# callmeray/PointMVSNet

Measured on AMD Instinct MI355X. Metric: depth-maps/sec (DTU 640x512, 3 src views, 2 flow iters), higher is better.
Workload: dtype f32

## Files before the change

### pointmvsnet_amd/csrc/conv2d_wide.hip

```cpp
#include <stdlib.h>

#include "pf_common.h"
#include "pf_bn_resolve.h"

namespace {

typedef float f32x16 __attribute__((ext_vector_type(16)));
typedef float f32x4 __attribute__((ext_vector_type(4)));
typedef float f32x2 __attribute__((ext_vector_type(2)));

struct WideGeom {
  int Hi, Wi, Ho, Wo, tiles_w, tiles_h, sps;
  int cl_out;
  int sets, spset, x_mode;
  int64_t w_stride;
};

__device__ __forceinline__ int wide_set(const WideGeom& g, int n) { return (g.sets > 1 && n >= g.spset) ? 1 : 0; }
__device__ __forceinline__ int wide_input_sample(const WideGeom& g, int n, int set) {
  const int i = n - set * g.spset;
  return g.x_mode == 0 ? n : (g.x_mode == 1 ? i : i * g.sets + set);
}

template <int KS, int STRIDE, int CIN, int COUT>
struct WideCfg {
  static constexpr int NWN = COUT / 32;
  static constexpr int NWM = 4 / NWN;
  static constexpr int TH = 2 * NWM, TW = 16;
  static constexpr int PAD = KS / 2;
  static constexpr int PH = (TH - 1) * STRIDE + KS, PW = (TW - 1) * STRIDE + KS;
  static constexpr int NPIX = PH * PW;
  static constexpr int RS = CIN + 4;
  static constexpr int PATCH = NPIX * RS;
  static constexpr int KC = CIN / 8;
  static constexpr size_t LDS = sizeof(float) * (size_t)(PATCH + 2 * CIN) + sizeof(double) * 4 * 32 * 2;
  static_assert(COUT == 32 || COUT == 64, "C_out is 32 or 64");
  static_assert(CIN % 8 == 0 && PATCH % 4 == 0, "16-byte pieces");
  static_assert(PATCH * sizeof(float) >= 4096, "pf_bn_resolve's scratch lives in the (still empty) patch");
  static_assert(LDS <= 80 * 1024, "two blocks per CU");
};

template <int CIN, int NPIX, int PW, int RS>
struct PatchStager {
  static constexpr int ITEMS = NPIX * ((CIN + 3) / 4);
  static constexpr int NIT = (ITEMS + 255) / 256;
  static constexpr int PH = NPIX / PW;
  static_assert(CIN % 4 == 0 || CIN < 4, "a padded quad: one quad only");
  static_assert(PH < 256 && PW < 256, "patch coordinates are packed in bytes");
  float rx[NIT][4];
  int goff[NIT];
  int meta[NIT];
  unsigned okmask;
  bool interior;

  __device__ __forceinline__ void init(int plane_i, int Wi) {
    const int tid = threadIdx.x;
#pragma unroll
    for (int r = 0; r < NIT; ++r) {
      const int it = tid + 256 * r;
      const int itc = it < ITEMS ? it : ITEMS - 1;
      const int q = itc / NPIX, p = itc - q * NPIX;
      const int pr = p / PW, pc = p - pr * PW;
      goff[r] = 4 * q * plane_i + pr * Wi + pc;
      meta[r] = pr | (pc << 8) | (q << 16);
    }
  }

  __device__ __forceinline__ void load(const float* __restrict__ xb, int plane_i, int ih0, int iw0, int Hi, int Wi) {
    interior = ih0 >= 0 && iw0 >= 0 && ih0 + PH <= Hi && iw0 + PW <= Wi;
    const int origin = ih0 * Wi + iw0;
    if (interior) {
      okmask = ~0u;
#pragma unroll
      for (int r = 0; r < NIT; ++r) {
        const float* src = xb + (goff[r] + origin);
#pragma unroll
        for (int j = 0; j < 4; ++j) rx[r][j] = (CIN % 4 == 0 || j < CIN) ? src[j * plane_i] : 0.0f;
      }
      return;
    }
    okmask = 0;
#pragma unroll
    for (int r = 0; r < NIT; ++r) {
      const int pr = meta[r] & 255, pc = (meta[r] >> 8) & 255, q = meta[r] >> 16;
      const int ih = ih0 + pr, iw = iw0 + pc;
      const bool ok = ih >= 0 && ih < Hi && iw >= 0 && iw < Wi;
      okmask |= (ok ? 1u : 0u) << r;
      const float* src = xb + (ok ? goff[r] + origin : 4 * q * plane_i);
#pragma unroll
      for (int j = 0; j < 4; ++j) rx[r][j] = (CIN % 4 == 0 || j < CIN) ? src[j * plane_i] : 0.0f;
    }
  }

  template <bool AFF>
  __device__ __forceinline__ void commit(float* patch, const float* aff) const {
    const int tid = threadIdx.x;
#pragma unroll
    for (int r = 0; r < NIT; ++r) {
      const int it = tid + 256 * r;
      const int pr = meta[r] & 255, pc = (meta[r] >> 8) & 255, q = meta[r] >> 16;
      f32x4 v = {rx[r][0], rx[r][1], rx[r][2], rx[r][3]};
      if (AFF) {
        const f32x4 a = *reinterpret_cast<const f32x4*>(aff + 4 * q);
        const f32x4 b = *reinterpret_cast<const f32x4*>(aff + CIN + 4 * q);
#pragma unroll
        for (int j = 0; j < 4; ++j) v[j] = fmaxf(fmaf(v[j], a[j], b[j]), 0.0f);
      }
      if (!interior && !((okmask >> r) & 1u)) v = (f32x4){0.0f, 0.0f, 0.0f, 0.0f};
      if (256 * (r + 1) <= ITEMS || it < ITEMS) *reinterpret_cast<f32x4*>(patch + (pr * PW + pc) * RS + 4 * q) = v;
    }
  }
};

template <int CIN, int AFFINE>
__device__ __forceinline__ void wide_affine_prologue(float* aff, const float* __restrict__ in_scale,
                                                     const float* __restrict__ in_shift, int stat,
                                                     const pf_bn_job& in_bn, double* scratch) {
  static_assert(CIN % 4 == 0 || AFFINE == 0, "a padded channel quad takes no affine");
  const int tid = threadIdx.x;
  if (AFFINE == 1) {
    const float* sc = in_scale + (int64_t)stat * CIN;
    const float* sh = in_shift + (int64_t)stat * CIN;
    if (tid < CIN) aff[tid] = sc[tid];
    else if (tid < 2 * CIN) aff[tid] = sh[tid - CIN];
    __syncthreads();
  }
  if (AFFINE == 2) pf_bn_resolve<256>(in_bn, stat, aff, aff + CIN, scratch);
}

template <int CIN, int NPIX, int PW, int RS, int AFFINE>
__device__ __forceinline__ void wide_stage_patch(const float* __restrict__ xb, int plane_i, int ih0, int iw0, int Hi,
                                                 int Wi, float* patch, float* aff, const float* __restrict__ in_scale,
                                                 const float* __restrict__ in_shift, int stat, const pf_bn_job& in_bn,
                                                 double* scratch) {
  PatchStager<CIN, NPIX, PW, RS> st;
  st.init(plane_i, Wi);
  st.load(xb, plane_i, ih0, iw0, Hi, Wi);
  wide_affine_prologue<CIN, AFFINE>(aff, in_scale, in_shift, stat, in_bn, scratch);
  st.template commit<(AFFINE != 0)>(patch, aff);
}

template <class C, int COUT>
__device__ __forceinline__ void wide_epilogue(const f32x16& acc, float* __restrict__ y, const WideGeom& g,
                                              double* __restrict__ partials, double* red, int n, int bx, int oh0,
                                              int ow0, int wm, int wn, int wave, int m, int h, int tid, bool cl_out) {
  const int co = wn * 32 + m;
  float* yb = y + ((int64_t)n * COUT + co) * ((int64_t)g.Ho * g.Wo);
  const bool vec_ok = (g.Wo & 3) == 0;
  float s = 0.0f, q = 0.0f;
  if (cl_out) {
    float* ycl = y + (int64_t)n * g.Ho * g.Wo * COUT + co;
#pragma unroll
    for (int rq = 0; rq < 4; ++rq) {
      const int oh = oh0 + 2 * wm + (rq >> 1);
      const int ow = ow0 + (rq & 1) * 8 + 4 * h;
      if (oh < g.Ho) {
#pragma unroll
        for (int e = 0; e < 4; ++e) {
          if (ow + e < g.Wo) {
            ycl[((int64_t)oh * g.Wo + ow + e) * COUT] = acc[4 * rq + e];
            s += acc[4 * rq + e];
            q += acc[4 * rq + e] * acc[4 * rq + e];
          }
        }
      }
    }
  } else
#pragma unroll
  for (int rq = 0; rq < 4; ++rq) {
    const int oh = oh0 + 2 * wm + (rq >> 1);
    const int ow = ow0 + (rq & 1) * 8 + 4 * h;
    if (oh < g.Ho) {
      float* dst = yb + (int64_t)oh * g.Wo + ow;
      if (vec_ok && ow + 3 < g.Wo) {
        *reinterpret_cast<float4*>(dst) = make_float4(acc[4 * rq], acc[4 * rq + 1], acc[4 * rq + 2], acc[4 * rq + 3]);
#pragma unroll
        for (int e = 0; e < 4; ++e) {
          s += acc[4 * rq + e];
          q += acc[4 * rq + e] * acc[4 * rq + e];
        }
      } else {
#pragma unroll
        for (int e = 0; e < 4; ++e) {
          if (ow + e < g.Wo) {
            dst[e] = acc[4 * rq + e];
            s += acc[4 * rq + e];
            q += acc[4 * rq + e] * acc[4 * rq + e];
          }
        }
      }
    }
  }
  if (partials != nullptr) {
    s += __shfl_xor(s, 32);
    q += __shfl_xor(q, 32);
    if (h == 0) {
      red[(wave * 32 + m) * 2 + 0] = (double)s;
      red[(wave * 32 + m) * 2 + 1] = (double)q;
    }
    __syncthreads();
    if (tid < COUT) {
      const int cn = tid >> 5, cm = tid & 31;
      double ds = 0.0, dq = 0.0;
#pragma unroll
      for (int w = 0; w < C::NWM; ++w) {
        ds += red[((w * C::NWN + cn) * 32 + cm) * 2 + 0];
        dq += red[((w * C::NWN + cn) * 32 + cm) * 2 + 1];
      }
      double* o = partials + (((int64_t)n * gridDim.x + bx) * COUT + tid) * 2;
      o[0] = ds;
      o[1] = dq;
    }
  }
}


template <int KS, int STRIDE, int CIN, int COUT, int AFFINE>
__global__ __launch_bounds__(256) void conv2d_wide_kernel(const float* __restrict__ x, const float* __restrict__ wp,
                                                            float* __restrict__ y, WideGeom g,
                                                            const float* __restrict__ in_scale,
                                                            const float* __restrict__ in_shift,
                                                            double* __restrict__ partials, pf_bn_job in_bn,
                                                            pf_bn_job in_bn1) {
  using C = WideCfg<KS, STRIDE, CIN, COUT>;
  constexpr int PW = C::PW, RS = C::RS, NPIX = C::NPIX;
  extern __shared__ __attribute__((aligned(16))) float lds[];
  float* patch = lds;
  float* aff = lds + C::PATCH;
  double* red = reinterpret_cast<double*>(aff + 2 * CIN);

  const int tid = threadIdx.x;
  const int wave = __builtin_amdgcn_readfirstlane(tid >> 6), lane = tid & 63;
  const int m = lane & 31, h = lane >> 5;
  const int wm = wave / C::NWN, wn = wave % C::NWN;
  unsigned xb_, xn_;
  pf_xcd_xy(xb_, xn_);
  const int n = (int)xn_, bx = (int)xb_;
  const int tw = bx % g.tiles_w, th = bx / g.tiles_w;
  const int oh0 = th * C::TH, ow0 = tw * C::TW;
  const int ih0 = oh0 * STRIDE - C::PAD, iw0 = ow0 * STRIDE - C::PAD;
  const int plane_i = g.Hi * g.Wi;
  const int set = wide_set(g, n);
  const float* xb = x + (int64_t)wide_input_sample(g, n, set) * CIN * plane_i;

  constexpr int NP = KS * KS * C::KC;
  constexpr int D = 6;
  const f32x4* bg = reinterpret_cast<const f32x4*>(wp + set * g.w_stride) + (h * COUT + wn * 32 + m);
  f32x4 bq[D];
#pragma unroll
  for (int d = 0; d < D; ++d) bq[d] = bg[(d < NP ? d : 0) * 2 * COUT];

  wide_stage_patch<CIN, NPIX, PW, RS, AFFINE>(xb, plane_i, ih0, iw0, g.Hi, g.Wi, patch, aff, in_scale, in_shift,
                                              AFFINE == 2 ? (n - set * g.spset) / g.sps : n / g.sps,
                                              set ? in_bn1 : in_bn, reinterpret_cast<double*>(patch));
  __syncthreads();

  f32x16 acc;
#pragma unroll
  for (int i = 0; i < 16; ++i) acc[i] = 0.0f;
  const float* abase = patch + ((2 * wm + (m >> 4)) * STRIDE * PW + (m & 15) * STRIDE) * RS + 4 * h;
  f32x4 a = *reinterpret_cast<const f32x4*>(abase);
#pragma unroll
  for (int t = 0; t < NP; ++t) {
    f32x4 an = a;
    if (t + 1 < NP) {
      const int tap = (t + 1) / C::KC, kc = (t + 1) % C::KC;
      const int kh = tap / KS, kw = tap % KS;
      an = *reinterpret_cast<const f32x4*>(abase + (kh * PW + kw) * RS + 8 * kc);
    }
    const f32x4 b = bq[t % D];
    __builtin_amdgcn_sched_barrier(0);
    acc = __builtin_amdgcn_mfma_f32_32x32x2f32(a.x, b.x, acc, 0, 0, 0);
    acc = __builtin_amdgcn_mfma_f32_32x32x2f32(a.y, b.y, acc, 0, 0, 0);
    acc = __builtin_amdgcn_mfma_f32_32x32x2f32(a.z, b.z, acc, 0, 0, 0);
    acc = __builtin_amdgcn_mfma_f32_32x32x2f32(a.w, b.w, acc, 0, 0, 0);
    __builtin_amdgcn_sched_barrier(0);
    if (t + D < NP) bq[t % D] = bg[(t + D) * 2 * COUT];
    a = an;
  }
  wide_epilogue<C, COUT>(acc, y, g, partials, red, n, bx, oh0, ow0, wm, wn, wave, m, h, tid, (g.cl_out >> set) & 1);
}

template <int KS, int STRIDE, int CIN, int COUT, int AFFINE>
int launch_wide_mode(const float* x, const float* wp, float* y, WideGeom g, int64_t N, const float* in_scale,
                     const float* in_shift, double* partials, const pf_bn_job& in_bn, const pf_bn_job& in_bn1,
                     hipStream_t s) {
  using C = WideCfg<KS, STRIDE, CIN, COUT>;
  if (C::LDS > 64 * 1024) {
    static std::atomic<unsigned long long> done{0};
    const int rc = pf_allow_big_lds(reinterpret_cast<const void*>(&conv2d_wide_kernel<KS, STRIDE, CIN, COUT, AFFINE>),
                                    (int)C::LDS, done);
    if (rc != PF_OK) return rc;
  }
  g.tiles_w = (g.Wo + C::TW - 1) / C::TW;
  const int tiles_h = (g.Ho + C::TH - 1) / C::TH;
  dim3 grid((unsigned)(tiles_h * g.tiles_w), (unsigned)N);
  hipLaunchKernelGGL((conv2d_wide_kernel<KS, STRIDE, CIN, COUT, AFFINE>), grid, dim3(256), C::LDS, s, x, wp, y, g,
                     in_scale, in_shift, partials, in_bn, in_bn1);
  return pf_launch_status();
}

template <int KS, int STRIDE, int CIN, int COUT>
int launch_wide(const float* x, const float* wp, float* y, WideGeom g, int64_t N, const float* in_scale,
                const float* in_shift, double* partials, const pf_bn_job* in_bn, hipStream_t s) {
  if (in_bn != nullptr) {
    for (int k = 0; k < g.sets; ++k) {
      const int rc = pf_bn_in_check(in_bn + k, CIN, g.spset / g.sps);
      if (rc != PF_OK) return rc;
    }
    return launch_wide_mode<KS, STRIDE, CIN, COUT, 2>(x, wp, y, g, N, nullptr, nullptr, partials, in_bn[0],
                                                      in_bn[g.sets - 1], s);
  }
  pf_bn_job none = {};
  if (in_scale != nullptr)
    return launch_wide_mode<KS, STRIDE, CIN, COUT, 1>(x, wp, y, g, N, in_scale, in_shift, partials, none, none, s);
  return launch_wide_mode<KS, STRIDE, CIN, COUT, 0>(x, wp, y, g, N, nullptr, nullptr, partials, none, none, s);
}

template <int KS, int STRIDE, int CIN, int COUT>
struct Wide16Cfg {
  static constexpr int TH = 16, TW = 16, NCOL = 16;
  static constexpr int PAD = KS / 2;
  static constexpr int PH = (TH - 1) * STRIDE + KS, PW = (TW - 1) * STRIDE + KS;
  static constexpr int NPIX = PH * PW;
  static constexpr int CINP = (CIN + 3) / 4 * 4;
  static constexpr int RS = CINP + 4;
  static constexpr int PATCH = NPIX * RS;
  static constexpr int CPL = CINP / 4;
  static constexpr bool PAIR = COUT == 8 && CIN >= 8;
  static constexpr int KH = PAIR ? KS + 1 : KS;
  static constexpr int WALL = KH * KS * CINP * NCOL;
  static constexpr int WSPACE = WALL > 1024 ? WALL : 1024;
  static constexpr size_t LDS = sizeof(float) * (size_t)(PATCH + WSPACE + 2 * CINP) + sizeof(double) * 4 * 16 * 2;
  static_assert(CIN == 3 || CIN == 8 || CIN == 16, "C_in is 3, 8 or 16");
  static_assert(COUT == 8 || COUT == 16, "C_out is 8 or 16");
  static_assert(!PAIR || STRIDE == 1, "paired rows: stride 1");
  static_assert(PATCH % 4 == 0 && WALL % 4 == 0, "16-byte pieces");
  static_assert(LDS <= 80 * 1024, "two blocks per CU");
};

template <int KS, int STRIDE, int CIN, int COUT, int AFFINE>
__global__ __launch_bounds__(256) void conv2d_wide16_kernel(const float* __restrict__ x, const float* __restrict__ wp,
                                                            float* __restrict__ y, WideGeom g,
                                                            const float* __restrict__ in_scale,
                                                            const float* __restrict__ in_shift,
                                                            double* __restrict__ partials, pf_bn_job in_bn,
                                                            pf_bn_job in_bn1) {
  using C = Wide16Cfg<KS, STRIDE, CIN, COUT>;
  constexpr int PW = C::PW, RS = C::RS, NPIX = C::NPIX, CPL = C::CPL, NCOL = 16;
  extern __shared__ __attribute__((aligned(16))) float lds[];
  float* patch = lds;
  float* wl = lds + C::PATCH;
  float* aff = wl + C::WSPACE;
  double* red = reinterpret_cast<double*>(aff + 2 * C::CINP);

  const int tid = threadIdx.x;
  const int wave = __builtin_amdgcn_readfirstlane(tid >> 6), lane = tid & 63;
  const int li = lane & 15, kq = lane >> 4;
  unsigned xb_, xn_;
  pf_xcd_xy(xb_, xn_);
  const int n = (int)xn_, bx = (int)xb_;
  const int plane_i = g.Hi * g.Wi;
  const int set = wide_set(g, n);
  const float* xb = x + (int64_t)wide_input_sample(g, n, set) * CIN * plane_i;
  wp += set * g.w_stride;
  const int tiles = g.tiles_h * g.tiles_w;
  const int nb = gridDim.x;

  constexpr int W4 = C::WALL / 4, NWR = (W4 + 255) / 256;
  f32x4 rw[NWR];
#pragma unroll
  for (int r = 0; r < NWR; ++r) {
    const int e = tid + 256 * r;
    rw[r] = reinterpret_cast<const f32x4*>(wp)[e < W4 ? e : W4 - 1];
  }
  PatchStager<CIN, NPIX, PW, RS> st;
  st.init(plane_i, g.Wi);
  int tile = bx;
  auto tile_origin = [&](int t, int& oh0, int& ow0) {
    const int th = t / g.tiles_w;
    oh0 = th * C::TH;
    ow0 = (t - th * g.tiles_w) * C::TW;
  };
  {
    int oh0, ow0;
    tile_origin(tile, oh0, ow0);
    st.load(xb, plane_i, oh0 * STRIDE - C::PAD, ow0 * STRIDE - C::PAD, g.Hi, g.Wi);
  }
  wide_affine_prologue<CIN, AFFINE>(aff, in_scale, in_shift, AFFINE == 2 ? (n - set * g.spset) / g.sps : n / g.sps,
                                    set ? in_bn1 : in_bn, reinterpret_cast<double*>(wl));
#pragma unroll
  for (int r = 0; r < NWR; ++r) {
    const int e = tid + 256 * r;
    if (256 * (r + 1) <= W4 || e < W4) reinterpret_cast<f32x4*>(wl)[e] = rw[r];
  }

  constexpr bool PAIR = C::PAIR;
  constexpr int NR = PAIR ? 2 : 4;
  const float* abase = patch + ((4 * wave) * STRIDE * PW + li * STRIDE) * RS + CPL * kq;
  const float* bbase = wl + (kq * NCOL + li) * CPL;
  constexpr int TAPS = C::KH * KS;
  struct Op {
    float v[CPL];
  };
  auto read_op = [&](const float* p) {
    Op o;
    if (CPL == 4) {
      const f32x4 t = *reinterpret_cast<const f32x4*>(p);
      o.v[0] = t[0];
      o.v[1 % CPL] = t[1];
      o.v[2 % CPL] = t[2];
      o.v[3 % CPL] = t[3];
    } else if (CPL == 2) {
      const f32x2 t = *reinterpret_cast<const f32x2*>(p);
      o.v[0] = t[0];
      o.v[1 % CPL] = t[1];
    } else {
      o.v[0] = p[0];
    }
    return o;
  };
  auto read_a = [&](int t, Op* a) {
    const int kh = t / KS, kw = t - kh * KS;
#pragma unroll
    for (int r = 0; r < NR; ++r) a[r] = read_op(abase + (((PAIR ? 2 * r : r) * STRIDE + kh) * PW + kw) * RS);
  };
  const bool vec_ok = (g.Wo & 3) == 0;
  const int my_co = PAIR ? (li & 7) : li;
  const int my_row = PAIR ? (li >> 3) : 0;
  const bool col_ok = my_co < COUT;
  const int plane_o = g.Ho * g.Wo;
  float* const yn = y + (int64_t)n * COUT * plane_o;
  double ds = 0.0, dq = 0.0;
#pragma unroll 1
  for (; tile < tiles; tile += nb) {
    int oh0, ow0;
    tile_origin(tile, oh0, ow0);
    st.template commit<(AFFINE != 0)>(patch, aff);
    __syncthreads();
    if (tile + nb < tiles) {
      int noh0, now0;
      tile_origin(tile + nb, noh0, now0);
      st.load(xb, plane_i, noh0 * STRIDE - C::PAD, now0 * STRIDE - C::PAD, g.Hi, g.Wi);
    }
    f32x4 acc[NR];
#pragma unroll
    for (int r = 0; r < NR; ++r) acc[r] = (f32x4){0.0f, 0.0f, 0.0f, 0.0f};
    Op a[NR], b;
    read_a(0, a);
    b = read_op(bbase);
#pragma unroll
    for (int t = 0; t < TAPS; ++t) {
      Op an[NR], bn = b;
#pragma unroll
      for (int r = 0; r < NR; ++r) an[r] = a[r];
      if (t + 1 < TAPS) {
        read_a(t + 1, an);
        bn = read_op(bbase + (t + 1) * 4 * NCOL * CPL);
      }
      __builtin_amdgcn_sched_barrier(0);
#pragma unroll
      for (int j = 0; j < CPL; ++j)
#pragma unroll
        for (int r = 0; r < NR; ++r) acc[r] = __builtin_amdgcn_mfma_f32_16x16x4f32(a[r].v[j], b.v[j], acc[r], 0, 0, 0);
      __builtin_amdgcn_sched_barrier(0);
#pragma unroll
      for (int r = 0; r < NR; ++r) a[r] = an[r];
      b = bn;
    }
    float s = 0.0f, q = 0.0f;
    const int ow = ow0 + 4 * kq;
    if (vec_ok && oh0 + C::TH <= g.Ho && ow0 + C::TW <= g.Wo) {
      float* dst = yn + (my_co * plane_o + (oh0 + 4 * wave + my_row) * g.Wo + ow);
      if (col_ok) {
#pragma unroll
        for (int r = 0; r < NR; ++r) {
          *reinterpret_cast<f32x4*>(dst + (PAIR ? 2 * r : r) * g.Wo) = acc[r];
#pragma unroll
          for (int e = 0; e < 4; ++e) {
            s += acc[r][e];
            q += acc[r][e] * acc[r][e];
          }
        }
      }
    } else {
      float* yb = yn + (int64_t)my_co * plane_o;
#pragma unroll
      for (int r = 0; r < NR; ++r) {
        const int oh = oh0 + 4 * wave + (PAIR ? 2 * r : r) + my_row;
        if (oh < g.Ho && col_ok) {
          float* dst = yb + (int64_t)oh * g.Wo + ow;
#pragma unroll
          for (int e = 0; e < 4; ++e) {
            if (ow + e < g.Wo) {
              dst[e] = acc[r][e];
              s += acc[r][e];
              q += acc[r][e] * acc[r][e];
            }
          }
        }
      }
    }
    ds += (double)s;
    dq += (double)q;
    __syncthreads();
  }
  if (PAIR && partials != nullptr) {
    ds += __shfl_xor(ds, 8);
    dq += __shfl_xor(dq, 8);
  }
  if (partials != nullptr) {
    ds += __shfl_xor(ds, 16);
    dq += __shfl_xor(dq, 16);
    ds += __shfl_xor(ds, 32);
    dq += __shfl_xor(dq, 32);
    if (lane < 16) {
      red[(wave * 16 + lane) * 2 + 0] = ds;
      red[(wave * 16 + lane) * 2 + 1] = dq;
    }
    __syncthreads();
    if (tid < COUT) {
      double ts = 0.0, tq = 0.0;
#pragma unroll
      for (int w = 0; w < 4; ++w) {
        ts += red[(w * 16 + tid) * 2 + 0];
        tq += red[(w * 16 + tid) * 2 + 1];
      }
      double* o = partials + (((int64_t)n * gridDim.x + bx) * COUT + tid) * 2;
      o[0] = ts;
      o[1] = tq;
    }
  }
}

#ifndef PF_W16_TPB
#define PF_W16_TPB 4
#endif
int wide16_blocks(int tiles) { return (tiles + PF_W16_TPB - 1) / PF_W16_TPB; }

template <int KS, int STRIDE, int CIN, int COUT, int AFFINE>
int launch_wide16_mode(const float* x, const float* wp, float* y, WideGeom g, int64_t N, const float* in_scale,
                       const float* in_shift, double* partials, const pf_bn_job& in_bn, const pf_bn_job& in_bn1,
                       hipStream_t s) {
  using C = Wide16Cfg<KS, STRIDE, CIN, COUT>;
  if (C::LDS > 64 * 1024) {
    static std::atomic<unsigned long long> done{0};
    const int rc = pf_allow_big_lds(
        reinterpret_cast<const void*>(&conv2d_wide16_kernel<KS, STRIDE, CIN, COUT, AFFINE>), (int)C::LDS, done);
    if (rc != PF_OK) return rc;
  }
  g.tiles_w = (g.Wo + C::TW - 1) / C::TW;
  g.tiles_h = (g.Ho + C::TH - 1) / C::TH;
  dim3 grid((unsigned)wide16_blocks(g.tiles_h * g.tiles_w), (unsigned)N);
  hipLaunchKernelGGL((conv2d_wide16_kernel<KS, STRIDE, CIN, COUT, AFFINE>), grid, dim3(256), C::LDS, s, x, wp, y, g,
                     in_scale, in_shift, partials, in_bn, in_bn1);
  return pf_launch_status();
}

template <int KS, int STRIDE, int CIN, int COUT>
int launch_wide16(const float* x, const float* wp, float* y, WideGeom g, int64_t N, const float* in_scale,
                  const float* in_shift, double* partials, const pf_bn_job* in_bn, hipStream_t s) {
  pf_bn_job none = {};
  if constexpr (CIN % 4 == 0) {
    if (in_bn != nullptr) {
      for (int k = 0; k < g.sets; ++k) {
        const int rc = pf_bn_in_check(in_bn + k, CIN, g.spset / g.sps);
        if (rc != PF_OK) return rc;
      }
      return launch_wide16_mode<KS, STRIDE, CIN, COUT, 2>(x, wp, y, g, N, nullptr, nullptr, partials, in_bn[0],
                                                          in_bn[g.sets - 1], s);
    }
    if (in_scale != nullptr)
      return launch_wide16_mode<KS, STRIDE, CIN, COUT, 1>(x, wp, y, g, N, in_scale, in_shift, partials, none, none, s);
  } else {
    if (in_bn != nullptr || in_scale != nullptr) return PF_ERR_UNSUPPORTED;
  }
  return launch_wide16_mode<KS, STRIDE, CIN, COUT, 0>(x, wp, y, g, N, nullptr, nullptr, partials, none, none, s);
}

int wide_tile_rows(int64_t Cout) { return Cout == 64 ? 4 : (Cout == 32 ? 8 : 16); }

}

extern "C" {

int pf_conv2d_wide_supported(int64_t Cin, int64_t Cout, int kernel_size, int stride) {
  if (kernel_size == 3 && stride == 1)
    return (Cin == 64 && Cout == 64) || (Cin == 32 && Cout == 32) || (Cin == 16 && Cout == 16) || (Cin == 8 && Cout == 8) ||
           (Cin == 3 && (Cout == 8 || Cout == 16));
  if (kernel_size == 5 && stride == 2) return (Cin == 32 && Cout == 64) || (Cin == 16 && Cout == 32) || (Cin == 8 && Cout == 16);
  return 0;
}

int pf_conv2d_wide_blocks(int64_t Cout, int64_t Hi, int64_t Wi, int stride) {
  if ((Cout != 8 && Cout != 16 && Cout != 32 && Cout != 64) || Hi <= 0 || Wi <= 0 || (stride != 1 && stride != 2)) return 0;
  const int64_t Ho = (Hi - 1) / stride + 1, Wo = (Wi - 1) / stride + 1;
  const int th = wide_tile_rows(Cout);
  const int tiles = (int)(((Ho + th - 1) / th) * ((Wo + 15) / 16));
  return Cout <= 16 ? wide16_blocks(tiles) : tiles;
}

int pf_conv2d_wide_f32(const float* x, const float* wp, float* y, int64_t N, int64_t Cin, int64_t Cout, int64_t Hi,
                       int64_t Wi, int kernel_size, int stride, const float* in_scale, const float* in_shift,
                       const pf_bn_job* in_bn, int samples_per_stat, double* partials, int out_channel_last,
                       void* stream) {
  return pf_conv2d_wide_sets_f32(x, 0, wp, 0, 1, y, N, Cin, Cout, Hi, Wi, kernel_size, stride, in_scale, in_shift, in_bn,
                                 samples_per_stat, partials, out_channel_last ? 1 : 0, stream);
}

int pf_conv2d_wide_sets_f32(const float* x, int x_layout, const float* wp, int64_t wp_set_stride, int sets, float* y,
                            int64_t N, int64_t Cin, int64_t Cout, int64_t Hi, int64_t Wi, int kernel_size, int stride,
                            const float* in_scale, const float* in_shift, const pf_bn_job* in_bn, int samples_per_stat,
                            double* partials, int out_channel_last, void* stream) {
  PF_REQUIRE(N >= 0 && Cin >= 1 && Cout >= 1 && Hi >= 1 && Wi >= 1 && N <= 65535 && samples_per_stat >= 1);
  PF_REQUIRE((sets == 1 || sets == 2) && N % sets == 0 && wp_set_stride >= 0 && (wp_set_stride & 3) == 0);
  PF_REQUIRE(out_channel_last >= 0 && out_channel_last < (1 << sets) && x_layout >= 0 && x_layout <= 2);
  if (out_channel_last && Cout < 32) return PF_ERR_UNSUPPORTED;
  PF_REQUIRE((in_scale == nullptr) == (in_shift == nullptr) && (in_bn == nullptr || in_scale == nullptr));
  PF_REQUIRE((N / sets) % samples_per_stat == 0 || (in_bn == nullptr && sets == 1));
  if (!pf_conv2d_wide_supported(Cin, Cout, kernel_size, stride)) return PF_ERR_UNSUPPORTED;
  PF_REQUIRE(Cin * Hi * Wi <= INT32_MAX);
  if (N == 0) return PF_OK;
  PF_REQUIRE(x && wp && y);
  WideGeom g;
  g.Hi = (int)Hi;
  g.Wi = (int)Wi;
  g.Ho = (int)((Hi - 1) / stride + 1);
  g.Wo = (int)((Wi - 1) / stride + 1);
  g.tiles_w = g.tiles_h = 0;
  g.sps = samples_per_stat;
  g.cl_out = out_channel_last;
  g.sets = sets;
  g.spset = (int)(N / sets);
  g.x_mode = sets > 1 ? x_layout : 0;
  g.w_stride = wp_set_stride;
  hipStream_t s = (hipStream_t)stream;
  if (Cout == 8) {
    if (Cin == 3) return launch_wide16<3, 1, 3, 8>(x, wp, y, g, N, in_scale, in_shift, partials, in_bn, s);
    return launch_wide16<3, 1, 8, 8>(x, wp, y, g, N, in_scale, in_shift, partials, in_bn, s);
  }
  if (Cout == 16) {
    if (Cin == 3) return launch_wide16<3, 1, 3, 16>(x, wp, y, g, N, in_scale, in_shift, partials, in_bn, s);
    if (kernel_size == 3) return launch_wide16<3, 1, 16, 16>(x, wp, y, g, N, in_scale, in_shift, partials, in_bn, s);
    return launch_wide16<5, 2, 8, 16>(x, wp, y, g, N, in_scale, in_shift, partials, in_bn, s);
  }
  if (kernel_size == 3) {
    if (Cin == 64) return launch_wide<3, 1, 64, 64>(x, wp, y, g, N, in_scale, in_shift, partials, in_bn, s);
    return launch_wide<3, 1, 32, 32>(x, wp, y, g, N, in_scale, in_shift, partials, in_bn, s);
  }
  if (Cin == 32) return launch_wide<5, 2, 32, 64>(x, wp, y, g, N, in_scale, in_shift, partials, in_bn, s);
  return launch_wide<5, 2, 16, 32>(x, wp, y, g, N, in_scale, in_shift, partials, in_bn, s);
}

}
```

Baseline: 1099.

## De-interleave stride-2 patch columns and shrink single-quad row stride in wide16 LDS patch

For the wide16 conv kernel, the LDS patch now stores stride-2 columns split into even and odd halves, so adjacent lanes read consecutive slots instead of every other column. This is meant to reduce LDS bank conflicts. For single-quad inputs the row stride drops from 8 to 6 floats, with each quad written as two 8-byte halves. The stager precomputes patch offsets, batches affine loads, and specialises commit for interior versus padded tiles. Sched barriers are inserted between stride-2 operand reads, which may limit how the compiler interleaves instructions.

```diff
diff --git a/pointmvsnet_amd/csrc/conv2d_wide.hip b/pointmvsnet_amd/csrc/conv2d_wide.hip
--- a/pointmvsnet_amd/csrc/conv2d_wide.hip
+++ b/pointmvsnet_amd/csrc/conv2d_wide.hip
@@ -32,6 +32,9 @@
   static constexpr int NPIX = PH * PW;
   static constexpr int RS = CIN + 4;
   static constexpr int PATCH = NPIX * RS;
+  static constexpr int SPLIT = 0;
+  static constexpr bool WALKS = false;
+  static __device__ __forceinline__ int patch_offset(int pr, int pc, int q) { return (pr * PW + pc) * RS + 4 * q; }
   static constexpr int KC = CIN / 8;
   static constexpr size_t LDS = sizeof(float) * (size_t)(PATCH + 2 * CIN) + sizeof(double) * 4 * 32 * 2;
   static_assert(COUT == 32 || COUT == 64, "C_out is 32 or 64");
@@ -40,7 +43,7 @@
   static_assert(LDS <= 80 * 1024, "two blocks per CU");
 };
 
-template <int CIN, int NPIX, int PW, int RS>
+template <int CIN, int NPIX, int PW, class L>
 struct PatchStager {
   static constexpr int ITEMS = NPIX * ((CIN + 3) / 4);
   static constexpr int NIT = (ITEMS + 255) / 256;
@@ -50,6 +53,7 @@
   float rx[NIT][4];
   int goff[NIT];
   int meta[NIT];
+  int poff[NIT];
   unsigned okmask;
   bool interior;
 
@@ -63,6 +67,7 @@
       const int pr = p / PW, pc = p - pr * PW;
       goff[r] = 4 * q * plane_i + pr * Wi + pc;
       meta[r] = pr | (pc << 8) | (q << 16);
+      if (L::WALKS) poff[r] = L::patch_offset(pr, pc, q);
     }
   }
 
@@ -92,23 +97,51 @@
     }
   }
 
+  template <bool AFF, bool PADDED>
+  __device__ __forceinline__ void commit_items(float* patch, const float* aff) const {
+    const int tid = threadIdx.x;
+    constexpr int CH = L::WALKS ? 4 : 1;
+#pragma unroll
+    for (int r0 = 0; r0 < NIT; r0 += CH) {
+      f32x4 a[CH], b[CH];
+      if (AFF) {
+#pragma unroll
+        for (int c = 0; c < CH; ++c) {
+          if (r0 + c < NIT) {
+            const int q = meta[r0 + c] >> 16;
+            a[c] = *reinterpret_cast<const f32x4*>(aff + 4 * q);
+            b[c] = *reinterpret_cast<const f32x4*>(aff + CIN + 4 * q);
+          }
+        }
+      }
+#pragma unroll
+      for (int c = 0; c < CH; ++c) {
+        const int r = r0 + c;
+        if (r < NIT) {
+          f32x4 v = {rx[r][0], rx[r][1], rx[r][2], rx[r][3]};
+          if (AFF) {
+#pragma unroll
+            for (int j = 0; j < 4; ++j) v[j] = fmaxf(fmaf(v[j], a[c][j], b[c][j]), 0.0f);
+          }
+          if (PADDED && !((okmask >> r) & 1u)) v = (f32x4){0.0f, 0.0f, 0.0f, 0.0f};
+          if (256 * (r + 1) <= ITEMS || tid + 256 * r < ITEMS) {
+            float* dst = patch + (L::WALKS ? poff[r] : L::patch_offset(meta[r] & 255, (meta[r] >> 8) & 255, meta[r] >> 16));
+            if (L::SPLIT == 0) {
+              *reinterpret_cast<f32x4*>(dst) = v;
+            } else {
+              *reinterpret_cast<f32x2*>(dst) = (f32x2){v[0], v[1]};
+              *reinterpret_cast<f32x2*>(dst + L::SPLIT) = (f32x2){v[2], v[3]};
+            }
+          }
+        }
+      }
+    }
+  }
+
   template <bool AFF>
   __device__ __forceinline__ void commit(float* patch, const float* aff) const {
-    const int tid = threadIdx.x;
-#pragma unroll
-    for (int r = 0; r < NIT; ++r) {
-      const int it = tid + 256 * r;
-      const int pr = meta[r] & 255, pc = (meta[r] >> 8) & 255, q = meta[r] >> 16;
-      f32x4 v = {rx[r][0], rx[r][1], rx[r][2], rx[r][3]};
-      if (AFF) {
-        const f32x4 a = *reinterpret_cast<const f32x4*>(aff + 4 * q);
-        const f32x4 b = *reinterpret_cast<const f32x4*>(aff + CIN + 4 * q);
-#pragma unroll
-        for (int j = 0; j < 4; ++j) v[j] = fmaxf(fmaf(v[j], a[j], b[j]), 0.0f);
-      }
-      if (!interior && !((okmask >> r) & 1u)) v = (f32x4){0.0f, 0.0f, 0.0f, 0.0f};
-      if (256 * (r + 1) <= ITEMS || it < ITEMS) *reinterpret_cast<f32x4*>(patch + (pr * PW + pc) * RS + 4 * q) = v;
-    }
+    if (interior) commit_items<AFF, false>(patch, aff);
+    else commit_items<AFF, true>(patch, aff);
   }
 };
 
@@ -128,12 +161,12 @@
   if (AFFINE == 2) pf_bn_resolve<256>(in_bn, stat, aff, aff + CIN, scratch);
 }
 
-template <int CIN, int NPIX, int PW, int RS, int AFFINE>
+template <int CIN, int NPIX, int PW, class L, int AFFINE>
 __device__ __forceinline__ void wide_stage_patch(const float* __restrict__ xb, int plane_i, int ih0, int iw0, int Hi,
                                                  int Wi, float* patch, float* aff, const float* __restrict__ in_scale,
                                                  const float* __restrict__ in_shift, int stat, const pf_bn_job& in_bn,
                                                  double* scratch) {
-  PatchStager<CIN, NPIX, PW, RS> st;
+  PatchStager<CIN, NPIX, PW, L> st;
   st.init(plane_i, Wi);
   st.load(xb, plane_i, ih0, iw0, Hi, Wi);
   wide_affine_prologue<CIN, AFFINE>(aff, in_scale, in_shift, stat, in_bn, scratch);
@@ -250,9 +283,9 @@
 #pragma unroll
   for (int d = 0; d < D; ++d) bq[d] = bg[(d < NP ? d : 0) * 2 * COUT];
 
-  wide_stage_patch<CIN, NPIX, PW, RS, AFFINE>(xb, plane_i, ih0, iw0, g.Hi, g.Wi, patch, aff, in_scale, in_shift,
-                                              AFFINE == 2 ? (n - set * g.spset) / g.sps : n / g.sps,
-                                              set ? in_bn1 : in_bn, reinterpret_cast<double*>(patch));
+  wide_stage_patch<CIN, NPIX, PW, C, AFFINE>(xb, plane_i, ih0, iw0, g.Hi, g.Wi, patch, aff, in_scale, in_shift,
+                                             AFFINE == 2 ? (n - set * g.spset) / g.sps : n / g.sps,
+                                             set ? in_bn1 : in_bn, reinterpret_cast<double*>(patch));
   __syncthreads();
 
   f32x16 acc;
@@ -324,9 +357,16 @@
   static constexpr int PH = (TH - 1) * STRIDE + KS, PW = (TW - 1) * STRIDE + KS;
   static constexpr int NPIX = PH * PW;
   static constexpr int CINP = (CIN + 3) / 4 * 4;
-  static constexpr int RS = CINP + 4;
+  static constexpr int CPL = CINP / 4;
+  static constexpr int RS = CPL == 1 ? 6 : CINP + 4;
+  static constexpr int HALF = (PW + 1) / 2;
   static constexpr int PATCH = NPIX * RS;
-  static constexpr int CPL = CINP / 4;
+  static constexpr int SPLIT = RS % 4 != 0 ? 2 : 0;
+  static constexpr bool WALKS = true;
+  static __device__ __forceinline__ int column_slot(int pc) { return STRIDE == 2 ? (pc & 1) * HALF + (pc >> 1) : pc; }
+  static __device__ __forceinline__ int patch_offset(int pr, int pc, int q) {
+    return (pr * PW + column_slot(pc)) * RS + 4 * q;
+  }
   static constexpr bool PAIR = COUT == 8 && CIN >= 8;
   static constexpr int KH = PAIR ? KS + 1 : KS;
   static constexpr int WALL = KH * KS * CINP * NCOL;
@@ -374,7 +414,7 @@
     const int e = tid + 256 * r;
     rw[r] = reinterpret_cast<const f32x4*>(wp)[e < W4 ? e : W4 - 1];
   }
-  PatchStager<CIN, NPIX, PW, RS> st;
+  PatchStager<CIN, NPIX, PW, C> st;
   st.init(plane_i, g.Wi);
   int tile = bx;
   auto tile_origin = [&](int t, int& oh0, int& ow0) {
@@ -397,7 +437,7 @@
 
   constexpr bool PAIR = C::PAIR;
   constexpr int NR = PAIR ? 2 : 4;
-  const float* abase = patch + ((4 * wave) * STRIDE * PW + li * STRIDE) * RS + CPL * kq;
+  const float* abase = patch + ((4 * wave) * STRIDE * PW + li) * RS + CPL * kq;
   const float* bbase = wl + (kq * NCOL + li) * CPL;
   constexpr int TAPS = C::KH * KS;
   struct Op {
@@ -423,7 +463,10 @@
   auto read_a = [&](int t, Op* a) {
     const int kh = t / KS, kw = t - kh * KS;
 #pragma unroll
-    for (int r = 0; r < NR; ++r) a[r] = read_op(abase + (((PAIR ? 2 * r : r) * STRIDE + kh) * PW + kw) * RS);
+    for (int r = 0; r < NR; ++r) {
+      a[r] = read_op(abase + (((PAIR ? 2 * r : r) * STRIDE + kh) * PW + C::column_slot(kw)) * RS);
+      if (STRIDE == 2) __builtin_amdgcn_sched_barrier(0);
+    }
   };
   const bool vec_ok = (g.Wo & 3) == 0;
   const int my_co = PAIR ? (li & 7) : li;
```

After: 1099 (median of 3 runs). No clear change (+0.0%).
